# wolearyc/ramannoodle

Hardware: AMD Instinct MI355X
Metric: structures/sec (GNN polarizability eval) (higher is better)
Workload: dtype f32

## Files before the change

include/rn_potgnn.h:

```cpp
#ifndef RN_POTGNN_H
#define RN_POTGNN_H

#include <stddef.h>
#include <stdint.h>

#ifdef __cplusplus
extern "C" {
#endif

typedef enum rn_status {
  RN_OK = 0,
  RN_ERR_INVALID_ARGUMENT = -1,
  RN_ERR_UNSUPPORTED = -2,
  RN_ERR_NO_DEVICE = -3,
  RN_ERR_HIP = -4,
  RN_ERR_OUT_OF_MEMORY = -5
} rn_status;

typedef struct rn_potgnn rn_potgnn;

typedef struct rn_potgnn_config {
  int32_t num_atoms;
  int32_t num_edges;
  int32_t num_atom_types;
// ... 136 lines not shown
int rn_md_raman_partial(const double *increments, int64_t N, int G, const double *weights, int64_t K, int device,
                        size_t workspace_limit, double *intensities, int64_t num_bins);
int rn_md_raman_partial_device(const double *d_increments, int64_t N, int G, const double *weights, int64_t K,
                               int device, size_t workspace_limit, double *intensities, int64_t num_bins, void *stream);

int rn_md_raman_segments(const double *alpha, int64_t S, int64_t segment_steps, int64_t hop, const double *taper,
                         const double *weights, int64_t K, int average, int device, size_t workspace_limit,
                         double *intensities, int64_t num_bins);
int rn_md_raman_segments_device(const double *d_alpha, int64_t S, int64_t segment_steps, int64_t hop, const double *taper,
                                const double *weights, int64_t K, int average, int device, size_t workspace_limit,
                                double *intensities, int64_t num_bins, void *stream);

int rn_md_raman_segments_at(const double *alpha, int64_t S, int64_t segment_steps, const int64_t *starts, int64_t Q,
                            const double *taper, const double *weights, int64_t K, int average, int device,
                            size_t workspace_limit, double *intensities, int64_t num_bins);
int rn_md_raman_segments_at_device(const double *d_alpha, int64_t S, int64_t segment_steps, const int64_t *starts,
                                   int64_t Q, const double *taper, const double *weights, int64_t K, int average,
                                   int device, size_t workspace_limit, double *intensities, int64_t num_bins,
                                   void *stream);

int rn_md_raman_partial_segments(const double *increments, int64_t N, int G, int64_t segment_steps,
                                 const int64_t *starts, int64_t Q, const double *taper, const double *weights,
                                 int64_t K, int average, int device, size_t workspace_limit, double *intensities,
                                 int64_t num_bins);
int rn_md_raman_partial_segments_device(const double *d_increments, int64_t N, int G, int64_t segment_steps,
                                        const int64_t *starts, int64_t Q, const double *taper, const double *weights,
                                        int64_t K, int average, int device, size_t workspace_limit,
                                        double *intensities, int64_t num_bins, void *stream);

int rn_md_vdos(const double *positions, const double *lattices, int64_t num_lattices, int64_t S, int32_t N,
               const double *masses, const int32_t *labels, int G, int64_t segment_steps, const int64_t *starts,
               int64_t Q, const double *taper, int average, int device, size_t workspace_limit, double *densities,
               int64_t num_bins);
int rn_md_vdos_device(const double *d_positions, const double *d_lattices, int64_t num_lattices, int64_t S, int32_t N,
                      const double *masses, const int32_t *labels, int G, int64_t segment_steps, const int64_t *starts,
                      int64_t Q, const double *taper, int average, int device, size_t workspace_limit,
                      double *densities, int64_t num_bins, void *stream);
int rn_md_vdos_set_profiling(int enabled);
int rn_md_vdos_phase_times(double *millis);

int rn_md_mode_vdos(const double *positions, const double *lattices, int64_t num_lattices, int64_t S, int32_t N,
                    const double *masses, const double *vectors, int32_t M, int64_t segment_steps,
                    const int64_t *starts, int64_t Q, const double *taper, int average, int device,
                    size_t workspace_limit, double *densities, int64_t num_bins);
int rn_md_mode_vdos_device(const double *d_positions, const double *d_lattices, int64_t num_lattices, int64_t S,
                           int32_t N, const double *masses, const double *vectors, int32_t M, int64_t segment_steps,
                           const int64_t *starts, int64_t Q, const double *taper, int average, int device,
                           size_t workspace_limit, double *densities, int64_t num_bins, void *stream);
int rn_md_mode_vdos_set_profiling(int enabled);
int rn_md_mode_vdos_phase_times(double *millis);

int rn_md_raman_modes(const double *increments, int64_t N, int C, int64_t segment_steps, const int64_t *starts,
                      int64_t Q, const double *taper, const double *weights, int64_t K, int average, int device,
                      size_t workspace_limit, double *intensities, int64_t num_bins);
int rn_md_raman_modes_device(const double *d_increments, int64_t N, int C, int64_t segment_steps, const int64_t *starts,
                             int64_t Q, const double *taper, const double *weights, int64_t K, int average, int device,
                             size_t workspace_limit, double *intensities, int64_t num_bins, void *stream);
int rn_md_raman_modes_set_profiling(int enabled);
int rn_md_raman_modes_phase_times(double *millis);

int rn_md_raman_mode_matrix(const double *increments, int64_t N, int C, int64_t segment_steps, const int64_t *starts,
                            int64_t Q, const double *taper, const double *weights, int64_t K, const double *bin_weights,
                            int64_t B, int device, size_t workspace_limit, double *matrices, int64_t num_bins);
int rn_md_raman_mode_matrix_device(const double *d_increments, int64_t N, int C, int64_t segment_steps,
                                   const int64_t *starts, int64_t Q, const double *taper, const double *weights,
                                   int64_t K, const double *bin_weights, int64_t B, int device, size_t workspace_limit,
                                   double *matrices, int64_t num_bins, void *stream);
int rn_md_raman_mode_matrix_set_profiling(int enabled);
int rn_md_raman_mode_matrix_phase_times(double *millis);
int rn_md_raman_mode_matrix_response(int64_t n, const double *bin_weights, int64_t B, int64_t num_bins, double scale,
                                     double *response);

int rn_potgnn_config_flags(const rn_potgnn *h);

int rn_potgnn_debug_ps_schedule(const int32_t *rb, const int32_t *re, int32_t num_destinations, int32_t back,
                                int32_t ring_tiles, int32_t *window);

int rn_potgnn_debug_plan(const rn_potgnn_config *cfg, const int32_t *edge_a, const int32_t *edge_b,
                         const int32_t *atom_types, int32_t num_cus, int32_t *out, size_t capacity, size_t *count);

int rn_potgnn_debug_plan_pairs(const rn_potgnn_config *cfg, const int32_t *edge_a, const int32_t *edge_b,
                               const int32_t *atom_types, int32_t num_cus, int32_t *out, size_t capacity, size_t *count);

int rn_potgnn_debug_plan_lds(const rn_potgnn_config *cfg, const int32_t *edge_a, const int32_t *edge_b,
                             const int32_t *atom_types, int32_t num_cus, int64_t *out, size_t capacity, size_t *count);

int rn_potgnn_debug_pack_weights(const rn_potgnn_config *cfg, const float *weights, size_t num_weights, float *packed,
                                 unsigned char *mask, unsigned char *writers, int32_t *flags, size_t capacity, size_t *count);

int rn_potgnn_debug_unpack_weights(const rn_potgnn_config *cfg, const float *packed, size_t num_packed, int buffers,
                                   float *out, size_t capacity, size_t *count);

int64_t rn_potgnn_num_triplets(const rn_potgnn *h);

int rn_potgnn_debug_triplets(rn_potgnn *h, int32_t *idx_i, int32_t *idx_j,
                             int32_t *idx_k, int32_t *slot5, int32_t *slot6);

int rn_potgnn_debug_stage(rn_potgnn *h, int stage, int index, float *out,
                          size_t out_capacity, int64_t *rows, int64_t *cols);

int rn_potgnn_set_profiling(rn_potgnn *h, int enabled);
int rn_potgnn_kernel_times(rn_potgnn *h, const char **names, double *millis,
                           int64_t *launches, int cap);

const char *rn_potgnn_last_error(const rn_potgnn *h);
const char *rn_potgnn_version(void);

#ifdef __cplusplus
}
#endif
#endif
```

ramannoodle_amd/_lib.py:

```python
from __future__ import annotations

import ctypes as C
import os

from ramannoodle_amd.exceptions import DeviceError

_LIB_PATH = os.environ.get(
    "RN_POTGNN_LIB", os.path.join(os.path.dirname(os.path.abspath(__file__)), "librn_potgnn.so"))

RN_OK = 0
RN_ERR_INVALID_ARGUMENT = -1
RN_ERR_UNSUPPORTED = -2
RN_ERR_NO_DEVICE = -3
RN_ERR_HIP = -4
RN_ERR_OUT_OF_MEMORY = -5


class Config(C.Structure):

    _fields_ = [
        ("num_atoms", C.c_int32),
        ("num_edges", C.c_int32),
        ("num_atom_types", C.c_int32),
        ("size_node_embedding", C.c_int32),
        ("size_edge_embedding", C.c_int32),
        ("num_message_passes", C.c_int32),
        ("gauss_coefficient", C.c_double),
        ("max_chunk_structures", C.c_int32),
        ("device", C.c_int32),
    ]


_P = C.c_void_p
SIGNATURES = {
    "rn_potgnn_radius_graph": (C.c_int, [_P, _P, C.c_int32, C.c_double, C.c_int, _P]),
    "rn_potgnn_config_flags": (C.c_int, [_P]),
    "rn_potgnn_set_stat_reducer": (C.c_int, [_P, _P, _P]),
    "rn_potgnn_train_row_count": (C.c_double, [_P]),
    "rn_potgnn_weight_count": (C.c_size_t, [C.POINTER(Config)]),
    "rn_potgnn_create": (C.c_int, [C.POINTER(Config), _P, _P, _P, _P, _P, C.c_size_t, _P, _P,
                                   C.POINTER(_P)]),
    "rn_potgnn_destroy": (None, [_P]),
    "rn_potgnn_calc_polarizabilities": (C.c_int, [_P, _P, C.c_int64, _P]),
    "rn_potgnn_calc_polarizabilities_f64": (C.c_int, [_P, _P, C.c_int64, _P]),
    "rn_potgnn_calc_polarizabilities_to_device": (C.c_int, [_P, _P, C.c_int64, _P, _P]),
    "rn_potgnn_calc_polarizabilities_cells": (C.c_int, [_P, _P, _P, C.c_int64, C.c_int, _P]),
    "rn_potgnn_calc_polarizabilities_cells_to_device": (C.c_int, [_P, _P, _P, C.c_int64, _P, _P]),
    "rn_potgnn_forward_cells_device": (C.c_int, [_P, _P, _P, C.c_int64, C.c_int, _P, _P, C.c_int]),
    "rn_potgnn_forward_device": (C.c_int, [_P, _P, C.c_int64, _P, _P, _P, C.c_int]),
    "rn_potgnn_forward_device_f64": (C.c_int, [_P, _P, C.c_int64, _P, _P, C.c_int]),
    "rn_potgnn_calc_polarizabilities_async": (C.c_int, [_P, _P, C.c_int64, _P]),
    "rn_potgnn_wait": (C.c_int, [_P]),
    "rn_host_buffer_alloc": (C.c_int, [C.c_size_t, C.c_int, C.POINTER(_P)]),
    "rn_host_buffer_free": (None, [_P]),
    "rn_potgnn_forward": (C.c_int, [_P, _P, C.c_int64, _P]),
    "rn_potgnn_forward_lattices": (C.c_int, [_P, _P, _P, C.c_int64, _P]),
    "rn_potgnn_forward_samples": (C.c_int, [_P, _P, _P, _P, C.c_int64, _P]),
    "rn_potgnn_forward_samples_f64": (C.c_int, [_P, _P, _P, _P, C.c_int64, _P]),
    "rn_potgnn_raman_tensors": (C.c_int, [_P, _P, _P, C.c_int64, C.c_double, _P]),
    "rn_potgnn_alpha_jacobian": (C.c_int, [_P, _P, C.c_int, _P]),
    "rn_potgnn_raman_tensors_analytic": (C.c_int, [_P, _P, _P, C.c_int64, _P]),
    "rn_potgnn_set_weights": (C.c_int, [_P, _P, C.c_size_t]),
    "rn_potgnn_train_forward": (C.c_int, [_P, _P, C.c_int64, _P, _P, _P]),
    "rn_potgnn_train_backward": (C.c_int, [_P, _P, _P]),
    "rn_potgnn_set_device_training": (C.c_int, [_P, C.c_int]),
    "rn_potgnn_train_backward_device": (C.c_int, [_P, _P]),
    "rn_potgnn_gradient_buffer": (C.c_int, [_P, C.POINTER(_P), C.POINTER(C.c_size_t)]),
    "rn_potgnn_adam_step": (C.c_int, [_P, C.c_double, C.c_double, C.c_double, C.c_double, C.c_double, C.c_int64]),
    "rn_potgnn_get_weights": (C.c_int, [_P, _P, C.c_size_t]),
    "rn_potgnn_train_forward_f64": (C.c_int, [_P, _P, C.c_int64, _P, _P, _P]),
    "rn_potgnn_train_forward_samples": (C.c_int, [_P, _P, _P, _P, C.c_int64, _P, _P, _P]),
    "rn_potgnn_train_forward_samples_f64": (C.c_int, [_P, _P, _P, _P, C.c_int64, _P, _P, _P]),
    "rn_potgnn_forward_samples_device": (C.c_int, [_P, _P, _P, _P, C.c_int64, _P, _P, C.c_int]),
    "rn_potgnn_train_forward_samples_device": (C.c_int, [_P, _P, _P, _P, C.c_int64, _P, _P]),
    "rn_potgnn_train_backward_samples_device": (C.c_int, [_P, _P, _P]),
    "rn_potgnn_train_backward_f64": (C.c_int, [_P, _P, _P]),
    "rn_potgnn_forward_vjp_device": (C.c_int, [_P, _P, _P, _P, C.c_int64, _P, C.c_int, _P, _P, _P]),
    "rn_potgnn_group_increments_device": (C.c_int, [_P, _P, C.c_int64, _P, C.c_int, C.c_int, C.c_size_t, _P, _P]),
    "rn_potgnn_group_increments_cells_device": (C.c_int, [_P, _P, _P, C.c_int64, _P, C.c_int, C.c_int, C.c_size_t, _P,
                                                          _P]),
    "rn_potgnn_partial_raman_tensors": (C.c_int, [_P, _P, _P, C.c_int64, _P, C.c_int, _P]),
    "rn_potgnn_mode_contract_device": (C.c_int, [_P, C.c_int64, _P, C.c_int32, _P, _P, C.c_int32, _P, C.c_int, C.c_int,
                                                 _P, _P]),
    "rn_potgnn_mode_increments_device": (C.c_int, [_P, _P, _P, C.c_int64, _P, _P, C.c_int32, C.c_int, C.c_int,
                                                   C.c_size_t, _P, _P]),
    "rn_potgnn_train_backward_inputs": (C.c_int, [_P, _P, _P, _P, _P]),
    "rn_potgnn_train_backward_inputs_device": (C.c_int, [_P, _P, _P, _P, _P]),
    "rn_potgnn_num_triplets": (C.c_int64, [_P]),
    "rn_potgnn_debug_triplets": (C.c_int, [_P, _P, _P, _P, _P, _P]),
    "rn_potgnn_debug_ps_schedule": (C.c_int, [_P, _P, C.c_int32, C.c_int32, C.c_int32, _P]),
    "rn_potgnn_debug_plan": (C.c_int, [C.POINTER(Config), _P, _P, _P, C.c_int32, _P, C.c_size_t, C.POINTER(C.c_size_t)]),
    "rn_potgnn_debug_plan_pairs": (C.c_int, [C.POINTER(Config), _P, _P, _P, C.c_int32, _P, C.c_size_t, C.POINTER(C.c_size_t)]),
    "rn_potgnn_debug_plan_lds": (C.c_int, [C.POINTER(Config), _P, _P, _P, C.c_int32, _P, C.c_size_t, C.POINTER(C.c_size_t)]),
    "rn_potgnn_debug_pack_weights": (C.c_int, [C.POINTER(Config), _P, C.c_size_t, _P, _P, _P, _P, C.c_size_t, C.POINTER(C.c_size_t)]),
    "rn_potgnn_debug_unpack_weights": (C.c_int, [C.POINTER(Config), _P, C.c_size_t, C.c_int, _P, C.c_size_t, C.POINTER(C.c_size_t)]),
    "rn_potgnn_debug_stage": (C.c_int, [_P, C.c_int, C.c_int, _P, C.c_size_t,
                                        C.POINTER(C.c_int64), C.POINTER(C.c_int64)]),
    "rn_potgnn_set_profiling": (C.c_int, [_P, C.c_int]),
    "rn_potgnn_kernel_times": (C.c_int, [_P, C.POINTER(C.c_char_p), C.POINTER(C.c_double),
                                         C.POINTER(C.c_int64), C.c_int]),
    "rn_potgnn_last_error": (C.c_char_p, [_P]),
    "rn_potgnn_version": (C.c_char_p, []),
    "rn_md_raman_intensities": (C.c_int, [_P, C.c_int64, C.c_int, _P, C.c_int64]),
    "rn_md_raman_intensities_device": (C.c_int, [_P, C.c_int64, C.c_int, _P, C.c_int64, _P]),
    "rn_md_raman_polarized": (C.c_int, [_P, C.c_int64, _P, C.c_int64, C.c_int, C.c_size_t, _P, C.c_int64]),
    "rn_md_raman_polarized_device": (C.c_int, [_P, C.c_int64, _P, C.c_int64, C.c_int, C.c_size_t, _P, C.c_int64,
                                               _P]),
    "rn_md_raman_partial": (C.c_int, [_P, C.c_int64, C.c_int, _P, C.c_int64, C.c_int, C.c_size_t, _P, C.c_int64]),
    "rn_md_raman_partial_device": (C.c_int, [_P, C.c_int64, C.c_int, _P, C.c_int64, C.c_int, C.c_size_t, _P,
                                             C.c_int64, _P]),
    "rn_md_raman_segments": (C.c_int, [_P, C.c_int64, C.c_int64, C.c_int64, _P, _P, C.c_int64, C.c_int, C.c_int,
                                       C.c_size_t, _P, C.c_int64]),
    "rn_md_raman_segments_device": (C.c_int, [_P, C.c_int64, C.c_int64, C.c_int64, _P, _P, C.c_int64, C.c_int, C.c_int,
                                              C.c_size_t, _P, C.c_int64, _P]),
    "rn_md_raman_segments_at": (C.c_int, [_P, C.c_int64, C.c_int64, _P, C.c_int64, _P, _P, C.c_int64, C.c_int, C.c_int,
                                          C.c_size_t, _P, C.c_int64]),
    "rn_md_raman_segments_at_device": (C.c_int, [_P, C.c_int64, C.c_int64, _P, C.c_int64, _P, _P, C.c_int64, C.c_int,
                                                 C.c_int, C.c_size_t, _P, C.c_int64, _P]),
    "rn_md_raman_partial_segments": (C.c_int, [_P, C.c_int64, C.c_int, C.c_int64, _P, C.c_int64, _P, _P, C.c_int64,
                                               C.c_int, C.c_int, C.c_size_t, _P, C.c_int64]),
    "rn_md_raman_partial_segments_device": (C.c_int, [_P, C.c_int64, C.c_int, C.c_int64, _P, C.c_int64, _P, _P,
                                                      C.c_int64, C.c_int, C.c_int, C.c_size_t, _P, C.c_int64, _P]),
    "rn_md_vdos": (C.c_int, [_P, _P, C.c_int64, C.c_int64, C.c_int32, _P, _P, C.c_int, C.c_int64, _P, C.c_int64, _P,
                             C.c_int, C.c_int, C.c_size_t, _P, C.c_int64]),
    "rn_md_vdos_device": (C.c_int, [_P, _P, C.c_int64, C.c_int64, C.c_int32, _P, _P, C.c_int, C.c_int64, _P, C.c_int64,
                                    _P, C.c_int, C.c_int, C.c_size_t, _P, C.c_int64, _P]),
    "rn_md_vdos_set_profiling": (C.c_int, [C.c_int]),
    "rn_md_vdos_phase_times": (C.c_int, [_P]),
    "rn_md_mode_vdos": (C.c_int, [_P, _P, C.c_int64, C.c_int64, C.c_int32, _P, _P, C.c_int32, C.c_int64, _P, C.c_int64,
                                  _P, C.c_int, C.c_int, C.c_size_t, _P, C.c_int64]),
    "rn_md_mode_vdos_device": (C.c_int, [_P, _P, C.c_int64, C.c_int64, C.c_int32, _P, _P, C.c_int32, C.c_int64, _P,
                                         C.c_int64, _P, C.c_int, C.c_int, C.c_size_t, _P, C.c_int64, _P]),
    "rn_md_mode_vdos_set_profiling": (C.c_int, [C.c_int]),
    "rn_md_mode_vdos_phase_times": (C.c_int, [_P]),
    "rn_md_raman_modes": (C.c_int, [_P, C.c_int64, C.c_int, C.c_int64, _P, C.c_int64, _P, _P, C.c_int64, C.c_int, C.c_int,
                                    C.c_size_t, _P, C.c_int64]),
    "rn_md_raman_modes_device": (C.c_int, [_P, C.c_int64, C.c_int, C.c_int64, _P, C.c_int64, _P, _P, C.c_int64, C.c_int,
                                           C.c_int, C.c_size_t, _P, C.c_int64, _P]),
    "rn_md_raman_modes_set_profiling": (C.c_int, [C.c_int]),
    "rn_md_raman_modes_phase_times": (C.c_int, [_P]),
    "rn_md_raman_mode_matrix": (C.c_int, [_P, C.c_int64, C.c_int, C.c_int64, _P, C.c_int64, _P, _P, C.c_int64, _P,
                                          C.c_int64, C.c_int, C.c_size_t, _P, C.c_int64]),
    "rn_md_raman_mode_matrix_device": (C.c_int, [_P, C.c_int64, C.c_int, C.c_int64, _P, C.c_int64, _P, _P, C.c_int64, _P,
                                                 C.c_int64, C.c_int, C.c_size_t, _P, C.c_int64, _P]),
    "rn_md_raman_mode_matrix_set_profiling": (C.c_int, [C.c_int]),
    "rn_md_raman_mode_matrix_phase_times": (C.c_int, [_P]),
    "rn_md_raman_mode_matrix_response": (C.c_int, [C.c_int64, _P, C.c_int64, C.c_int64, C.c_double, _P]),
    "rn_xdatcar_open": (C.c_int, [C.c_char_p, C.POINTER(_P)]),
    "rn_xdatcar_close": (None, [_P]),
    "rn_xdatcar_info": (C.c_int, [_P, C.POINTER(C.c_int64), C.POINTER(C.c_int32), _P, C.POINTER(C.c_int32)]),
    "rn_xdatcar_species": (C.c_int, [_P, C.c_int32, C.c_char_p, C.POINTER(C.c_int32)]),
    "rn_xdatcar_read": (C.c_int, [_P, C.c_int64, C.c_int64, _P, _P, C.c_int]),
    "rn_xdatcar_variable_cell": (C.c_int, [_P]),
    "rn_xdatcar_read_lattices": (C.c_int, [_P, C.c_int64, C.c_int64, _P]),
    "rn_xdatcar_last_error": (C.c_char_p, [_P]),
    "rn_vasprun_open": (C.c_int, [C.c_char_p, C.POINTER(_P)]),
    "rn_vasprun_close": (None, [_P]),
    "rn_vasprun_info": (C.c_int, [_P, C.POINTER(C.c_int64), C.POINTER(C.c_int32)]),
    "rn_vasprun_read": (C.c_int, [_P, C.c_int64, C.c_int64, _P, C.c_int]),
    "rn_vasprun_timestep": (C.c_int, [_P, C.POINTER(C.c_double)]),
    "rn_vasprun_initial_num_atoms": (C.c_int64, [_P]),
    "rn_vasprun_initial_structure": (C.c_int, [_P, C.POINTER(C.c_int32), _P, _P, C.c_int64, _P, C.c_int64]),
    "rn_vasprun_last_error": (C.c_char_p, [_P]),
}

INTERP_SIGNATURES = {
    "rn_interp_create": (C.c_int, [C.c_int32, _P, _P, _P, C.c_int32, _P, _P, _P, _P, _P, C.c_int, C.POINTER(_P)]),
    "rn_interp_destroy": (None, [_P]),
    "rn_interp_last_error": (C.c_char_p, [_P]),
    "rn_interp_set_mask": (C.c_int, [_P, _P]),
    "rn_interp_is_symmetric": (C.c_int, [_P]),
    "rn_interp_calc_polarizabilities": (C.c_int, [_P, _P, C.c_int64, _P]),
    "rn_interp_forward_device": (C.c_int, [_P, _P, C.c_int64, _P, _P]),
    "rn_interp_jacobian_device": (C.c_int, [_P, _P, C.c_int64, _P, _P]),
    "rn_interp_group_increments_device": (C.c_int, [_P, _P, C.c_int64, _P, C.c_int, C.c_size_t, _P, _P]),
# ... 68 lines not shown
```

ramannoodle_amd/csrc/api.hip:

```cpp
#include <hip/hip_runtime.h>

#include <algorithm>
#include <chrono>
#include <cmath>
#include <cstdarg>
#include <cstdio>
#include <cstdlib>
#include <cstring>
#include <functional>
#include <memory>
#include <mutex>
#include <string>
#include <thread>
#include <vector>

#include "../../include/rn_potgnn.h"
#include "graph_plan.hpp"
#include "host_runtime.hpp"
#include "increments.hpp"
#include "kernels.hpp"
#include "weight_layout.hpp"

using namespace rn;

namespace {

std::string g_create_error;

enum KernelId {
  K_GEOM = 0, K_NODE_INIT, K_PROJ_NODE, K_PROJ_EDGE_C1, K_NODE_AGG, K_PROJ_EDGE_C3, K_PROJ_C2,
  K_EDGE_AGG, K_READOUT_MLP, K_READOUT_REDUCE, K_C2_PAIRS, K_COUNT
};
const char *kKernelNames[K_COUNT] = {
    "geom_rbf", "node_init", "proj_node", "proj_edge_c1", "node_agg", "proj_edge_c3",
    "proj_c2", "edge_agg", "readout_mlp", "readout_reduce", "c2_pairs"};

template <typename T>
struct Lane {
  hipStream_t stream = nullptr;
  hipEvent_t done = nullptr;
  DeviceBuf unit4, node[2], edge[2], npc1, np3, bufA, bufB;
  DeviceBuf fbA, fbB;
};

template <typename T>
struct Precision {
  bool ready = false;
  DeviceBuf weights;
  DeviceBuf lattice;
  std::vector<PassW<T>> pass;
  ReadoutW<T> ro{};
  const T *offsets = nullptr, *node_table = nullptr, *ones = nullptr;
  Lane<T> lanes[2];
  std::vector<DeviceBuf> snap_node, snap_edge;
  std::vector<DeviceBuf> tape_node, tape_edge, tape_agg;
  DeviceBuf bw[18];
  hipStream_t side = nullptr;
  hipEvent_t ev_side[3] = {nullptr, nullptr, nullptr};
  DeviceBuf tn_arena;
  DeviceBuf tape_z1, bn_stats, grad, seeds, mv, type_sums;
  DeviceBuf in_dcart, in_lat, in_grads;
  DeviceBuf eye_seeds;
  int eye_frames = 0;
  bool tape_on = false;
};

struct TimedLaunch {
  int kid;
  hipEvent_t a, b;
};

}

struct rn_potgnn {
  mutable std::recursive_mutex lock;
  rn_potgnn_config cfg{};
  Dims d{};
  int chunk = 1;
  size_t f64_budget = 0;
  bool keep_stages = false;
  bool snap_pairs = false;
  bool last_pair_rows = false;
  bool debug_sync = false;
  GraphPlan plan;
  bool split_projections = true;
  bool want_pair_rows = true;
  bool want_c2_pairs = true;
  DeviceBuf step_seg, step_stage;
  float *step_host = nullptr;
  bool tape_ps = true;
  bool mfma_f16 = true;
  bool mfma_f16_requested = true;
  bool mfma_range_fallback = false;
  Graph g{};
  DeviceBuf g_ints;
  DeviceBuf ps_fail;
  double lattice[9], mean[9], stdv[9];
  DeviceBuf d_mean_std;
  std::vector<float> packed;
// ... 2427 lines not shown
}

int rn_potgnn_set_stat_reducer(rn_potgnn *h, rn_potgnn_reduce_fn fn, void *ctx) {
  if (!h) return RN_ERR_INVALID_ARGUMENT;
  std::lock_guard<std::recursive_mutex> hold(h->lock);
  h->reducer = fn;
  h->reducer_ctx = ctx;
  return RN_OK;
}

double rn_potgnn_train_row_count(const rn_potgnn *h) {
  if (!h) return 0.0;
  std::lock_guard<std::recursive_mutex> hold(h->lock);
  return h->bn_count;
}

int rn_potgnn_train_backward(rn_potgnn *h, const float *dvec6, float *grads) {
  const Checked c = check_pending(h, dvec6 && grads, "train_backward", kHostF32,
                                  "train_backward needs a preceding train_forward (an evaluation or Jacobian call in "
                                  "between discards its tape)");
  if (c.rc != kGo) return c.rc;
  return guarded(h, [&]() { train_backward<float>(h, dvec6, grads); });
}

int rn_potgnn_radius_graph(const double *lattice, const double *positions, int32_t num_atoms,
                           double cutoff, int device, uint8_t *adjacency) {
  if (!lattice || !positions || !adjacency || num_atoms <= 0 || !(cutoff > 0)) {
    set_error<rn_potgnn>(nullptr, "invalid arguments to radius_graph");
    return RN_ERR_INVALID_ARGUMENT;
  }
  int ndev = 0;
  if (hipGetDeviceCount(&ndev) != hipSuccess || device < 0 || device >= ndev) {
    set_error<rn_potgnn>(nullptr, "no usable HIP device (count=%d, requested=%d)", ndev, device);
    return RN_ERR_NO_DEVICE;
  }
  return guarded<rn_potgnn>(nullptr, [&]() {
    HIP_TRY(hipSetDevice(device));
    const size_t n = (size_t)num_atoms;
    DeviceBuf lat, pos, adj;
    lat.ensure(9 * sizeof(double));
    pos.ensure(n * 3 * sizeof(double));
    adj.ensure(n * n);
    HIP_TRY(hipMemcpy(lat.p, lattice, 9 * sizeof(double), hipMemcpyHostToDevice));
    HIP_TRY(hipMemcpy(pos.p, positions, n * 3 * sizeof(double), hipMemcpyHostToDevice));
    launch_radius_graph(lat.as<double>(), pos.as<double>(), num_atoms, (float)cutoff,
                        adj.as<unsigned char>(), nullptr);
    HIP_TRY(hipGetLastError());
    HIP_TRY(hipDeviceSynchronize());
    HIP_TRY(hipMemcpy(adjacency, adj.p, n * n, hipMemcpyDeviceToHost));
  });
}

int rn_potgnn_config_flags(const rn_potgnn *h) {
  if (!h) return -1;
  std::lock_guard<std::recursive_mutex> hold(h->lock);
  int flags = (h->plan.use_fused ? 1 : 0) | ((h->plan.use_fused && h->mfma_f16) ? 4 : 0) | (h->plan.use_narrow ? 8 : 0) |
              ((h->plan.use_fused && h->mfma_range_fallback) ? 16 : 0);
  {
    bool ps = h->plan.use_fused && h->plan.use_ps && !h->f32.pass.empty();
    for (const auto &p : h->f32.pass) ps = ps && (p.c3_fast & 1);
    flags |= ps ? 256 : 0;
  }
  {
    static const bool centred = !(getenv("RN_POTGNN_NODE_CENTRED") && atoi(getenv("RN_POTGNN_NODE_CENTRED")) == 0);
    const bool atom = h->plan.use_fused && h->plan.use_node_fused && h->mfma_f16 && centred && h->g.na_num > 0;
    flags |= atom ? 512 : 0;
    flags |= (atom && (flags & 256) && h->plan.use_readout_fused && h->want_pair_rows && !h->keep_stages) ? 1024 : 0;
    flags |= ((flags & 1024) && h->want_c2_pairs && c2_rows_fit(h)) ? 2048 : 0;
  }
  bool fast = !h->f32.pass.empty();
  for (const auto &p : h->f32.pass) fast = fast && !h->plan.use_narrow && (p.c3_fast & (h->plan.use_fused ? 1 : 2));
  return flags | (fast ? 2 : 0);
}

int rn_potgnn_debug_ps_schedule(const int32_t *rb, const int32_t *re, int32_t num_destinations, int32_t back, int32_t ring_tiles,
                                int32_t *window) {
  if (!rb || !re || num_destinations < 0 || back < 1 || back > 8 || ring_tiles < 1 || ring_tiles > 64) return RN_ERR_INVALID_ARGUMENT;
  int w = 0;
  const bool ok = edge_ps_tile_ok(rb, re, num_destinations, back, ring_tiles, &w);
  if (window) *window = w;
  return ok ? 1 : 0;
}

int64_t rn_potgnn_num_triplets(const rn_potgnn *h) { return h ? h->g.T : -1; }

int rn_potgnn_debug_triplets(rn_potgnn *h, int32_t *idx_i, int32_t *idx_j, int32_t *idx_k,
                             int32_t *slot5, int32_t *slot6) {
  if (!h || !idx_i || !idx_j || !idx_k || !slot5 || !slot6) return RN_ERR_INVALID_ARGUMENT;
  return guarded(h, [&]() {
    const size_t T = (size_t)h->g.T;
    if (T == 0) return;
    DeviceBuf buf;
    buf.ensure(5 * T * sizeof(int));
    int *p = buf.as<int>();
    launch_enum_triplets(h->g, p, p + T, p + 2 * T, p + 3 * T, p + 4 * T, nullptr);
    HIP_TRY(hipGetLastError());
    HIP_TRY(hipDeviceSynchronize());
    int32_t *outs[5] = {idx_i, idx_j, idx_k, slot5, slot6};
    for (int k = 0; k < 5; ++k)
      HIP_TRY(hipMemcpy(outs[k], p + k * T, T * sizeof(int), hipMemcpyDeviceToHost));
  });
}

int rn_potgnn_debug_stage(rn_potgnn *h, int stage, int index, float *out, size_t out_capacity,
                          int64_t *rows, int64_t *cols) {
  if (!h || !out || !rows || !cols) return RN_ERR_INVALID_ARGUMENT;
  std::lock_guard<std::recursive_mutex> hold(h->lock);
  if (h->last_was_f64) {
    set_error(h, "debug_stage only reads the float32 path");
    return RN_ERR_UNSUPPORTED;
  }
  const int S = h->last_chunk_structs;
  Precision<float> &P = h->f32;
  return guarded(h, [&]() {
    HIP_TRY(hipDeviceSynchronize());
    const float *src = nullptr;
    int64_t r = 0, c = 0, ld = 0;
    const int64_t ME = (int64_t)S * h->g.E, MN = (int64_t)S * h->g.N;
    if (stage == 0) {
      src = P.lanes[0].unit4.as<float>(); r = ME; c = 4; ld = 4;
    } else if (stage == 1 || stage == 2) {
      if ((!h->keep_stages && !h->snap_pairs) || index < 0 || index > h->cfg.num_message_passes)
        throw HipError{hipErrorInvalidValue, "stage snapshots need RN_POTGNN_KEEP_STAGES=1 or 2"};
      if (stage == 1) { src = P.snap_node[index].as<float>(); r = MN; c = h->d.Fn; ld = h->d.FnP; }
      else { src = P.snap_edge[index].as<float>(); r = ME; c = h->d.Fe; ld = h->d.FeP; }
    } else if (stage == 3) {
      src = P.lanes[0].bufA.as<float>(); r = ME; c = 12; ld = 32;
    } else {
      throw HipError{hipErrorInvalidValue, "unknown stage"};
    }
    if ((size_t)(r * c) > out_capacity) throw HipError{hipErrorInvalidValue, "out_capacity too small"};
    if (stage == 2 && h->snap_pairs && h->last_pair_rows) {
      std::vector<_Float16> raw((size_t)r * 128);
      HIP_TRY(hipMemcpy(raw.data(), src, raw.size() * sizeof(_Float16), hipMemcpyDeviceToHost));
      for (int64_t i = 0; i < r; ++i)
        for (int64_t k = 0; k < c; ++k) {
          const _Float16 *grp = raw.data() + i * 128 + (k >> 3) * 16;
          out[i * c + k] = (float)grp[k & 7] + (float)grp[8 + (k & 7)];
        }
      *rows = r;
      *cols = c;
      return;
    }
    HIP_TRY(hipMemcpy2D(out, c * sizeof(float), src, ld * sizeof(float), c * sizeof(float), r,
                        hipMemcpyDeviceToHost));
    if (h->last_in_order && r == ME && stage != 1) {
      std::vector<float> tmp(out, out + r * c);
      const int E = h->g.E;
      for (int64_t s = 0; s < S; ++s)
        for (int e = 0; e < E; ++e)
          std::memcpy(out + (s * E + e) * c, tmp.data() + (s * E + h->plan.in_pos[e]) * c, (size_t)c * sizeof(float));
    }
    *rows = r;
    *cols = c;
  });
}

int rn_potgnn_set_profiling(rn_potgnn *h, int enabled) {
  if (!h) return RN_ERR_INVALID_ARGUMENT;
  std::lock_guard<std::recursive_mutex> hold(h->lock);
  resolve_timers(h);
  h->profiling = enabled;
  for (int k = 0; k < K_COUNT; ++k) {
    h->k_ms[k] = 0;
    h->k_launches[k] = 0;
  }
// ... 20 lines not shown
```

ramannoodle_amd/csrc/kernels_c2_pairs.hip:

```cpp
#include "fused_common.hpp"

namespace rn {

struct C2PairArgs {
  const float *node;
  float *out;
  int64_t M;
  int N, NP;
  const int *pair_a, *pair_b;
  Dims d;
  PassW<float> w;
};

namespace {
constexpr int C2P_THREADS = 256;
}

__global__ __launch_bounds__(C2P_THREADS, 2) void c2_pairs_kernel(C2PairArgs a) {
  __shared__ __attribute__((aligned(16))) float s_bias[2 * FP], s_g1[2 * FP], s_b1[2 * FP], s_g2[FP], s_b2[FP];
  const int tid = threadIdx.x, lane = tid & 63, wave = tid >> 6;
  const int l15 = lane & 15, quad = lane >> 4;
  const float sc2 = a.w.mfma_scale_c[4];
  for (int c = tid; c < 2 * FP; c += C2P_THREADS) {
    s_bias[c] = a.w.c2_bias_c[c] * sc2;
    s_g1[c] = a.w.c2_norm_1.g[c];
    s_b1[c] = a.w.c2_norm_1.b[c];
    if (c < FP) {
      s_g2[c] = a.w.c2_norm_2.g[c];
      s_b2[c] = a.w.c2_norm_2.b[c];
    }
  }
  WaveB<true> bW[4];
#pragma unroll
  for (int p = 0; p < 4; ++p) bW[p].load(a.w.c2_WT_c, 2 * FP, 32 * p, l15, quad, sc2);
  __syncthreads();

  const float inv2n = 1.0f / (float)(2 * a.d.Fe), invn = 1.0f / (float)a.d.Fe;
  const float eps_c2 = 1e-5f * sc2 * sc2;
  const int64_t ntiles = (a.M + 15) / 16, stride = (int64_t)gridDim.x * (C2P_THREADS / 64);

  f32x4 xb[4], xa[4];
  auto fetch = [&](int64_t tile) {
    int64_t row = tile * 16 + l15;
    if (row >= a.M) row = a.M - 1;
    const int64_t s = row / a.NP;
    const int p = (int)(row - s * a.NP);
    const float *nb = a.node + (s * a.N + a.pair_b[p]) * FP + 16 * quad, *na = a.node + (s * a.N + a.pair_a[p]) * FP + 16 * quad;
#pragma unroll
    for (int j = 0; j < 4; ++j) {
      xb[j] = *reinterpret_cast<const f32x4 *>(nb + 4 * j);
      xa[j] = *reinterpret_cast<const f32x4 *>(na + 4 * j);
    }
  };
  int64_t tile = (int64_t)blockIdx.x * (C2P_THREADS / 64) + wave;
  if (tile < ntiles) fetch(tile);
  for (; tile < ntiles; tile += stride) {
    float af[KS];
#pragma unroll
    for (int j = 0; j < 4; ++j) {
      const f32x4 pr = xb[j] * xa[j];
#pragma unroll
      for (int i = 0; i < 4; ++i) af[4 * j + i] = pr[i];
    }
    f16x8 ah[2], al[2];
    split_f16x8(af, ah[0], al[0]);
    split_f16x8(af + 8, ah[1], al[1]);
    if (tile + stride < ntiles) fetch(tile + stride);

    const int lq = launder(lane >> 4);
    f32x4 acc[4][2];
#pragma unroll
    for (int p = 0; p < 4; ++p) {
#pragma unroll
      for (int t = 0; t < 2; ++t) acc[p][t] = *reinterpret_cast<const f32x4 *>(s_bias + 32 * p + 16 * t + 4 * lq);
      bW[p].product_split(ah, al, acc[p]);
    }
    float q = 0.f;
#pragma unroll
    for (int p = 0; p < 4; ++p)
#pragma unroll
      for (int t = 0; t < 2; ++t)
#pragma unroll
        for (int i = 0; i < 4; ++i) q = fmaf(acc[p][t][i], acc[p][t][i], q);
    q = sum_xor32(sum_xor16(q));
    const float rstd2 = fast_rsq(q * inv2n + eps_c2);
    float gv[2][2][4], sum = 0.f;
#pragma unroll
    for (int p = 0; p < 2; ++p)
#pragma unroll
      for (int t = 0; t < 2; ++t) {
        const int c = 32 * p + 16 * t + 4 * lq;
        const Vec4<float> gf = load4<float>(s_g1 + c), bf = load4<float>(s_b1 + c);
        const Vec4<float> gc = load4<float>(s_g1 + FP + c), bc = load4<float>(s_b1 + FP + c);
#pragma unroll
        for (int i = 0; i < 4; ++i) {
          gv[p][t][i] = gate(acc[p][t][i] * rstd2 * gf.v[i] + bf.v[i], acc[p + 2][t][i] * rstd2 * gc.v[i] + bc.v[i]);
          sum += gv[p][t][i];
        }
      }
    const float mean = sum_xor32(sum_xor16(sum)) * invn;
    float qq = 0.f;
#pragma unroll
    for (int p = 0; p < 2; ++p)
#pragma unroll
      for (int t = 0; t < 2; ++t)
#pragma unroll
        for (int i = 0; i < 4; ++i) {
          const int c = 32 * p + 16 * t + 4 * lq + i;
          gv[p][t][i] = c < a.d.Fe ? gv[p][t][i] - mean : 0.f;
          qq = fmaf(gv[p][t][i], gv[p][t][i], qq);
        }
    const float rstd = fast_rsq(sum_xor32(sum_xor16(qq)) * invn + 1e-5f);
    const int64_t row = tile * 16 + l15;
    if (row < a.M) {
#pragma unroll
      for (int p = 0; p < 2; ++p)
#pragma unroll
        for (int t = 0; t < 2; ++t) {
          const int c = 32 * p + 16 * t + 4 * lq;
          const Vec4<float> g2 = load4<float>(s_g2 + c), b2 = load4<float>(s_b2 + c);
          f32x4 y;
#pragma unroll
          for (int i = 0; i < 4; ++i) y[i] = gv[p][t][i] * rstd * g2.v[i] + b2.v[i];
          *reinterpret_cast<f32x4 *>(a.out + row * FP + c) = y;
        }
    }
  }
}

void launch_c2_pairs(const float *node, float *out, int S, const Graph &g, Dims d, const PassW<float> &w, hipStream_t st) {
  const int64_t M = (int64_t)S * g.NP;
  if (M == 0) return;
  C2PairArgs a{node, out, M, g.N, g.NP, g.pair_a, g.pair_b, d, w};
  static int cus = 0;
  if (cus == 0) {
    int dev = 0;
    hipDeviceProp_t prop;
    if (hipGetDevice(&dev) == hipSuccess && hipGetDeviceProperties(&prop, dev) == hipSuccess) cus = prop.multiProcessorCount;
    if (cus <= 0) cus = 256;
  }
  const int64_t ntiles = (M + 15) / 16, per_wg = C2P_THREADS / 64;
  const int64_t grid = std::min<int64_t>((ntiles + per_wg - 1) / per_wg, (int64_t)2 * cus);
  c2_pairs_kernel<<<(unsigned)grid, C2P_THREADS, 0, st>>>(a);
}

}
```

Before: 64900.

## Restructure c2 pair kernel to walk pair tiles across frames with multi-frame batching

The c2 pairs kernel now assigns each wave a fixed pair tile and walks it across frames, processing U frames per iteration. Pair indices and offsets are loaded once per tile instead of once per row, and bias loads are shared across the U frames. The kernel is also templated on whether feature padding is needed, so the masking compare is dropped when Fe equals FP. The grid is sized by a new placement function that spreads waves over XCD-like groups, and occupancy is set from U. The trade-off is higher register pressure (with U=2 the launch bound drops to one wave per SIMD) in exchange for more instruction-level parallelism and less index overhead.

```diff
diff --git a/include/rn_potgnn.h b/include/rn_potgnn.h
--- a/include/rn_potgnn.h
+++ b/include/rn_potgnn.h
@@ -242,6 +242,9 @@
 int rn_potgnn_debug_plan_pairs(const rn_potgnn_config *cfg, const int32_t *edge_a, const int32_t *edge_b,
                                const int32_t *atom_types, int32_t num_cus, int32_t *out, size_t capacity, size_t *count);
 
+int rn_potgnn_debug_c2_units(int32_t num_frames, int32_t num_pairs, int32_t waves, int32_t frames_in_flight, int32_t num_cus,
+                             int32_t *out, size_t capacity, size_t *count, int32_t *info);
+
 int rn_potgnn_debug_plan_lds(const rn_potgnn_config *cfg, const int32_t *edge_a, const int32_t *edge_b,
                              const int32_t *atom_types, int32_t num_cus, int64_t *out, size_t capacity, size_t *count);
 
diff --git a/ramannoodle_amd/_lib.py b/ramannoodle_amd/_lib.py
--- a/ramannoodle_amd/_lib.py
+++ b/ramannoodle_amd/_lib.py
@@ -91,6 +91,8 @@
     "rn_potgnn_debug_ps_schedule": (C.c_int, [_P, _P, C.c_int32, C.c_int32, C.c_int32, _P]),
     "rn_potgnn_debug_plan": (C.c_int, [C.POINTER(Config), _P, _P, _P, C.c_int32, _P, C.c_size_t, C.POINTER(C.c_size_t)]),
     "rn_potgnn_debug_plan_pairs": (C.c_int, [C.POINTER(Config), _P, _P, _P, C.c_int32, _P, C.c_size_t, C.POINTER(C.c_size_t)]),
+    "rn_potgnn_debug_c2_units": (C.c_int, [C.c_int32, C.c_int32, C.c_int32, C.c_int32, C.c_int32, _P, C.c_size_t,
+                                           C.POINTER(C.c_size_t), _P]),
     "rn_potgnn_debug_plan_lds": (C.c_int, [C.POINTER(Config), _P, _P, _P, C.c_int32, _P, C.c_size_t, C.POINTER(C.c_size_t)]),
     "rn_potgnn_debug_pack_weights": (C.c_int, [C.POINTER(Config), _P, C.c_size_t, _P, _P, _P, _P, C.c_size_t, C.POINTER(C.c_size_t)]),
     "rn_potgnn_debug_unpack_weights": (C.c_int, [C.POINTER(Config), _P, C.c_size_t, C.c_int, _P, C.c_size_t, C.POINTER(C.c_size_t)]),
diff --git a/ramannoodle_amd/csrc/api.hip b/ramannoodle_amd/csrc/api.hip
--- a/ramannoodle_amd/csrc/api.hip
+++ b/ramannoodle_amd/csrc/api.hip
@@ -15,6 +15,7 @@
 #include <vector>
 
 #include "../../include/rn_potgnn.h"
+#include "c2_pairs_units.hpp"
 #include "graph_plan.hpp"
 #include "host_runtime.hpp"
 #include "increments.hpp"
@@ -2608,6 +2609,40 @@
   return ok ? 1 : 0;
 }
 
+int rn_potgnn_debug_c2_units(int32_t num_frames, int32_t num_pairs, int32_t waves, int32_t frames_in_flight, int32_t num_cus,
+                             int32_t *out, size_t capacity, size_t *count, int32_t *info) {
+  const int U = frames_in_flight == 0 ? RN_C2P_U : frames_in_flight;
+  if (!count || num_frames < 1 || num_frames > (1 << 24) || num_pairs < 1 || num_pairs > (1 << 24) || waves < 0 ||
+      waves > (1 << 20) || U < 1 || U > C2P_MAX_U || num_cus <= 0 || num_cus > 4096)
+    return RN_ERR_INVALID_ARGUMENT;
+  const int W = waves == 0 ? c2_grid_waves(num_frames, num_pairs, num_cus, U) : waves;
+  if (info) {
+    info[0] = W;
+    info[1] = RN_C2P_U;
+    info[2] = c2p_waves_per_simd(U);
+  }
+  auto walk = [&](int32_t *dst) {
+    size_t n = 0;
+    C2Walk wk;
+    for (int w = 0; w < W; ++w)
+      for (int k = 0; c2_walk(num_frames, num_pairs, W, U, w, k, wk); ++k)
+        for (int64_t s = wk.s0; s < num_frames; s += wk.ds, ++n)
+          if (dst) {
+            dst[3 * n] = w;
+            dst[3 * n + 1] = wk.pt;
+            dst[3 * n + 2] = (int32_t)s;
+          }
+    return 3 * n;
+  };
+  *count = walk(nullptr);
+  if (!out || capacity < *count) {
+    set_error<rn_potgnn>(nullptr, "out holds %zu values, the walk has %zu", out ? capacity : (size_t)0, *count);
+    return RN_ERR_INVALID_ARGUMENT;
+  }
+  walk(out);
+  return RN_OK;
+}
+
 int64_t rn_potgnn_num_triplets(const rn_potgnn *h) { return h ? h->g.T : -1; }
 
 int rn_potgnn_debug_triplets(rn_potgnn *h, int32_t *idx_i, int32_t *idx_j, int32_t *idx_k,
diff --git a/ramannoodle_amd/csrc/c2_pairs_units.hpp b/ramannoodle_amd/csrc/c2_pairs_units.hpp
--- /dev/null
+++ b/ramannoodle_amd/csrc/c2_pairs_units.hpp
@@ -0,0 +1,50 @@
+#pragma once
+#include <cstdint>
+
+#ifndef RN_C2P_U
+#define RN_C2P_U 2
+#endif
+
+namespace rn {
+
+constexpr int C2P_MAX_U = 3;
+static_assert(RN_C2P_U >= 1 && RN_C2P_U <= C2P_MAX_U, "RN_C2P_U: 1, 2 or 3");
+constexpr int c2p_waves_per_simd(int U) { return U == 1 ? 2 : 1; }
+
+struct C2Walk {
+  int pt;
+  int s0;
+  int ds;
+};
+
+__host__ __device__ inline int c2_wave_place(int W, int w) {
+  if (W % 4 != 0) return w;
+  const int nb = W / 4, b = w / 4, q = nb / 8, r = nb % 8, x = b % 8;
+  const int vb = (x < r ? x * (q + 1) : r * (q + 1) + (x - r) * q) + b / 8;
+  return 4 * vb + w % 4;
+}
+
+__host__ __device__ inline bool c2_walk(int S, int NP, int W, int U, int w, int k, C2Walk &o) {
+  const int PT = (NP + 15) / 16, G = W >= PT ? W / PT : 1;
+  const int64_t v = (int64_t)c2_wave_place(W, w) + (int64_t)k * W;
+  if (PT == 0 || v >= (int64_t)PT * G) return false;
+  o.pt = (int)(v % PT);
+  const int64_t first = (v / PT) * U;
+  o.s0 = first < S ? (int)first : S;
+  o.ds = G * U;
+  return true;
+}
+
+inline int c2_grid_waves(int S, int NP, int cus, int U) {
+  const int64_t PT = ((int64_t)NP + 15) / 16, steps = ((int64_t)S + U - 1) / U;
+  const int64_t slots = (int64_t)cus * 4 * c2p_waves_per_simd(U);
+  int64_t W = slots;
+  if (PT < slots) {
+    int64_t G = slots / PT;
+    if (G > steps) G = steps;
+    W = PT * (G > 0 ? G : 1);
+  }
+  return (int)((W + 3) / 4 * 4);
+}
+
+}
diff --git a/ramannoodle_amd/csrc/kernels_c2_pairs.hip b/ramannoodle_amd/csrc/kernels_c2_pairs.hip
--- a/ramannoodle_amd/csrc/kernels_c2_pairs.hip
+++ b/ramannoodle_amd/csrc/kernels_c2_pairs.hip
@@ -1,3 +1,4 @@
+#include "c2_pairs_units.hpp"
 #include "fused_common.hpp"
 
 namespace rn {
@@ -5,8 +6,7 @@
 struct C2PairArgs {
   const float *node;
   float *out;
-  int64_t M;
-  int N, NP;
+  int S, N, NP;
   const int *pair_a, *pair_b;
   Dims d;
   PassW<float> w;
@@ -16,10 +16,13 @@
 constexpr int C2P_THREADS = 256;
 }
 
-__global__ __launch_bounds__(C2P_THREADS, 2) void c2_pairs_kernel(C2PairArgs a) {
+template <int U, bool PAD>
+__global__ __launch_bounds__(C2P_THREADS, c2p_waves_per_simd(U)) void c2_pairs_kernel(C2PairArgs a) {
   __shared__ __attribute__((aligned(16))) float s_bias[2 * FP], s_g1[2 * FP], s_b1[2 * FP], s_g2[FP], s_b2[FP];
-  const int tid = threadIdx.x, lane = tid & 63, wave = tid >> 6;
+  const int tid = threadIdx.x, lane = tid & 63;
   const int l15 = lane & 15, quad = lane >> 4;
+  const int w = __builtin_amdgcn_readfirstlane((int)blockIdx.x * (C2P_THREADS / 64) + (tid >> 6));
+  const int W = (int)gridDim.x * (C2P_THREADS / 64);
   const float sc2 = a.w.mfma_scale_c[4];
   for (int c = tid; c < 2 * FP; c += C2P_THREADS) {
     s_bias[c] = a.w.c2_bias_c[c] * sc2;
@@ -37,101 +40,137 @@
 
   const float inv2n = 1.0f / (float)(2 * a.d.Fe), invn = 1.0f / (float)a.d.Fe;
   const float eps_c2 = 1e-5f * sc2 * sc2;
-  const int64_t ntiles = (a.M + 15) / 16, stride = (int64_t)gridDim.x * (C2P_THREADS / 64);
+  const int S = a.S;
+  const int64_t node_frame = (int64_t)a.N * FP, out_frame = (int64_t)a.NP * FP;
 
-  f32x4 xb[4], xa[4];
-  auto fetch = [&](int64_t tile) {
-    int64_t row = tile * 16 + l15;
-    if (row >= a.M) row = a.M - 1;
-    const int64_t s = row / a.NP;
-    const int p = (int)(row - s * a.NP);
-    const float *nb = a.node + (s * a.N + a.pair_b[p]) * FP + 16 * quad, *na = a.node + (s * a.N + a.pair_a[p]) * FP + 16 * quad;
+  C2Walk wk;
+  for (int k = 0; c2_walk(S, a.NP, W, U, w, k, wk); ++k) {
+    const int pair = 16 * wk.pt + l15;
+    const bool real = pair < a.NP;
+    const int pc = real ? pair : a.NP - 1;
+    const unsigned off_b = (unsigned)(a.pair_b[pc] * FP + 16 * quad), off_a = (unsigned)(a.pair_a[pc] * FP + 16 * quad);
+    const unsigned off_o = (unsigned)(pair * FP);
+
+    f32x4 xb[U][4], xa[U][4];
+    auto fetch = [&](int s) {
 #pragma unroll
-    for (int j = 0; j < 4; ++j) {
-      xb[j] = *reinterpret_cast<const f32x4 *>(nb + 4 * j);
-      xa[j] = *reinterpret_cast<const f32x4 *>(na + 4 * j);
-    }
-  };
-  int64_t tile = (int64_t)blockIdx.x * (C2P_THREADS / 64) + wave;
-  if (tile < ntiles) fetch(tile);
-  for (; tile < ntiles; tile += stride) {
-    float af[KS];
+      for (int u = 0; u < U; ++u) {
+        const float *frame = a.node + (int64_t)(s + u < S ? s + u : S - 1) * node_frame;
 #pragma unroll
-    for (int j = 0; j < 4; ++j) {
-      const f32x4 pr = xb[j] * xa[j];
-#pragma unroll
-      for (int i = 0; i < 4; ++i) af[4 * j + i] = pr[i];
-    }
-    f16x8 ah[2], al[2];
-    split_f16x8(af, ah[0], al[0]);
-    split_f16x8(af + 8, ah[1], al[1]);
-    if (tile + stride < ntiles) fetch(tile + stride);
-
-    const int lq = launder(lane >> 4);
-    f32x4 acc[4][2];
-#pragma unroll
-    for (int p = 0; p < 4; ++p) {
-#pragma unroll
-      for (int t = 0; t < 2; ++t) acc[p][t] = *reinterpret_cast<const f32x4 *>(s_bias + 32 * p + 16 * t + 4 * lq);
-      bW[p].product_split(ah, al, acc[p]);
-    }
-    float q = 0.f;
-#pragma unroll
-    for (int p = 0; p < 4; ++p)
-#pragma unroll
-      for (int t = 0; t < 2; ++t)
-#pragma unroll
-        for (int i = 0; i < 4; ++i) q = fmaf(acc[p][t][i], acc[p][t][i], q);
-    q = sum_xor32(sum_xor16(q));
-    const float rstd2 = fast_rsq(q * inv2n + eps_c2);
-    float gv[2][2][4], sum = 0.f;
-#pragma unroll
-    for (int p = 0; p < 2; ++p)
-#pragma unroll
-      for (int t = 0; t < 2; ++t) {
-        const int c = 32 * p + 16 * t + 4 * lq;
-        const Vec4<float> gf = load4<float>(s_g1 + c), bf = load4<float>(s_b1 + c);
-        const Vec4<float> gc = load4<float>(s_g1 + FP + c), bc = load4<float>(s_b1 + FP + c);
-#pragma unroll
-        for (int i = 0; i < 4; ++i) {
-          gv[p][t][i] = gate(acc[p][t][i] * rstd2 * gf.v[i] + bf.v[i], acc[p + 2][t][i] * rstd2 * gc.v[i] + bc.v[i]);
-          sum += gv[p][t][i];
+        for (int j = 0; j < 4; ++j) {
+          xb[u][j] = *reinterpret_cast<const f32x4 *>(frame + off_b + 4 * j);
+          xa[u][j] = *reinterpret_cast<const f32x4 *>(frame + off_a + 4 * j);
         }
       }
-    const float mean = sum_xor32(sum_xor16(sum)) * invn;
-    float qq = 0.f;
+    };
+    int s = wk.s0;
+    if (s < S) fetch(s);
+    while (s < S) {
+      f16x8 ah[U][2], al[U][2];
 #pragma unroll
-    for (int p = 0; p < 2; ++p)
+      for (int u = 0; u < U; ++u) {
+        float af[KS];
 #pragma unroll
-      for (int t = 0; t < 2; ++t)
+        for (int j = 0; j < 4; ++j) {
+          const f32x4 pr = xb[u][j] * xa[u][j];
 #pragma unroll
-        for (int i = 0; i < 4; ++i) {
-          const int c = 32 * p + 16 * t + 4 * lq + i;
-          gv[p][t][i] = c < a.d.Fe ? gv[p][t][i] - mean : 0.f;
-          qq = fmaf(gv[p][t][i], gv[p][t][i], qq);
+          for (int i = 0; i < 4; ++i) af[4 * j + i] = pr[i];
         }
-    const float rstd = fast_rsq(sum_xor32(sum_xor16(qq)) * invn + 1e-5f);
-    const int64_t row = tile * 16 + l15;
-    if (row < a.M) {
+        split_f16x8(af, ah[u][0], al[u][0]);
+        split_f16x8(af + 8, ah[u][1], al[u][1]);
+      }
+      const bool more = S - s > wk.ds;
+      fetch(more ? s + wk.ds : s);
+
+      const int lq = launder(lane >> 4);
+      f32x4 acc[U][4][2];
+#pragma unroll
+      for (int p = 0; p < 4; ++p) {
+        f32x4 bias[2];
+#pragma unroll
+        for (int t = 0; t < 2; ++t) bias[t] = *reinterpret_cast<const f32x4 *>(s_bias + 32 * p + 16 * t + 4 * lq);
+#pragma unroll
+        for (int u = 0; u < U; ++u) {
+#pragma unroll
+          for (int t = 0; t < 2; ++t) acc[u][p][t] = bias[t];
+          bW[p].product_split(ah[u], al[u], acc[u][p]);
+        }
+      }
+      float rstd2[U];
+#pragma unroll
+      for (int u = 0; u < U; ++u) {
+        float q = 0.f;
+#pragma unroll
+        for (int p = 0; p < 4; ++p)
+#pragma unroll
+          for (int t = 0; t < 2; ++t)
+#pragma unroll
+            for (int i = 0; i < 4; ++i) q = fmaf(acc[u][p][t][i], acc[u][p][t][i], q);
+        q = sum_xor32(sum_xor16(q));
+        rstd2[u] = fast_rsq(q * inv2n + eps_c2);
+      }
+      float gv[U][2][2][4], sum[U];
+#pragma unroll
+      for (int u = 0; u < U; ++u) sum[u] = 0.f;
+#pragma unroll
+      for (int p = 0; p < 2; ++p)
+#pragma unroll
+        for (int t = 0; t < 2; ++t) {
+          const int c = 32 * p + 16 * t + 4 * lq;
+          const Vec4<float> gf = load4<float>(s_g1 + c), bf = load4<float>(s_b1 + c);
+          const Vec4<float> gc = load4<float>(s_g1 + FP + c), bc = load4<float>(s_b1 + FP + c);
+#pragma unroll
+          for (int u = 0; u < U; ++u)
+#pragma unroll
+            for (int i = 0; i < 4; ++i) {
+              gv[u][p][t][i] = gate(acc[u][p][t][i] * rstd2[u] * gf.v[i] + bf.v[i], acc[u][p + 2][t][i] * rstd2[u] * gc.v[i] + bc.v[i]);
+              sum[u] += gv[u][p][t][i];
+            }
+        }
+      float rstd[U];
+#pragma unroll
+      for (int u = 0; u < U; ++u) {
+        const float mean = sum_xor32(sum_xor16(sum[u])) * invn;
+        float qq = 0.f;
+#pragma unroll
+        for (int p = 0; p < 2; ++p)
+#pragma unroll
+          for (int t = 0; t < 2; ++t)
+#pragma unroll
+            for (int i = 0; i < 4; ++i) {
+              if constexpr (PAD) {
+                const int c = 32 * p + 16 * t + 4 * lq + i;
+                gv[u][p][t][i] = c < a.d.Fe ? gv[u][p][t][i] - mean : 0.f;
+              } else {
+                gv[u][p][t][i] = gv[u][p][t][i] - mean;
+              }
+              qq = fmaf(gv[u][p][t][i], gv[u][p][t][i], qq);
+            }
+        rstd[u] = fast_rsq(sum_xor32(sum_xor16(qq)) * invn + 1e-5f);
+      }
 #pragma unroll
       for (int p = 0; p < 2; ++p)
 #pragma unroll
         for (int t = 0; t < 2; ++t) {
           const int c = 32 * p + 16 * t + 4 * lq;
           const Vec4<float> g2 = load4<float>(s_g2 + c), b2 = load4<float>(s_b2 + c);
-          f32x4 y;
 #pragma unroll
-          for (int i = 0; i < 4; ++i) y[i] = gv[p][t][i] * rstd * g2.v[i] + b2.v[i];
-          *reinterpret_cast<f32x4 *>(a.out + row * FP + c) = y;
+          for (int u = 0; u < U; ++u) {
+            f32x4 y;
+#pragma unroll
+            for (int i = 0; i < 4; ++i) y[i] = gv[u][p][t][i] * rstd[u] * g2.v[i] + b2.v[i];
+            if (real && s + u < S) *reinterpret_cast<f32x4 *>(a.out + (int64_t)(s + u) * out_frame + (off_o + (unsigned)c)) = y;
+          }
         }
+      if (!more) break;
+      s += wk.ds;
     }
   }
 }
 
 void launch_c2_pairs(const float *node, float *out, int S, const Graph &g, Dims d, const PassW<float> &w, hipStream_t st) {
-  const int64_t M = (int64_t)S * g.NP;
-  if (M == 0) return;
-  C2PairArgs a{node, out, M, g.N, g.NP, g.pair_a, g.pair_b, d, w};
+  if (S <= 0 || g.NP <= 0) return;
+  C2PairArgs a{node, out, S, g.N, g.NP, g.pair_a, g.pair_b, d, w};
   static int cus = 0;
   if (cus == 0) {
     int dev = 0;
@@ -139,9 +178,11 @@
     if (hipGetDevice(&dev) == hipSuccess && hipGetDeviceProperties(&prop, dev) == hipSuccess) cus = prop.multiProcessorCount;
     if (cus <= 0) cus = 256;
   }
-  const int64_t ntiles = (M + 15) / 16, per_wg = C2P_THREADS / 64;
-  const int64_t grid = std::min<int64_t>((ntiles + per_wg - 1) / per_wg, (int64_t)2 * cus);
-  c2_pairs_kernel<<<(unsigned)grid, C2P_THREADS, 0, st>>>(a);
+  const unsigned grid = (unsigned)(c2_grid_waves(S, g.NP, cus, RN_C2P_U) / (C2P_THREADS / 64));
+  if (d.Fe < FP)
+    c2_pairs_kernel<RN_C2P_U, true><<<grid, C2P_THREADS, 0, st>>>(a);
+  else
+    c2_pairs_kernel<RN_C2P_U, false><<<grid, C2P_THREADS, 0, st>>>(a);
 }
 
 }
```

Result: no change. 65290 (median of 6 runs) (+0.6%).
